# CWBudde/algo-dsp

Hardware: AMD Instinct MI355X
Metric: Msamples/sec, overlap-save conv 131072-tap IR @48kHz; achieved HBM GB/s (higher is better)
Workload: dtype f64

## Files before the change

### algo-dsp_amd/csrc/conv_long_kernels.hip

```cpp
#include "conv_long_kernels.hpp"

#include "conv_kernels.hpp"
#include "fft_device.hpp"

namespace adsp {

constexpr int N1 = kLongN1, N2 = kLongN2, W = kLongW;
constexpr int kColThreads = 256;
constexpr int kRowsPerInstr = kColThreads / W;
constexpr int FS = N1 + 1;
using ColPlan = FftPlan<N1, 16>;
constexpr int RV = 8;
using RowPlan = FftPlan<N2, RV>;
static_assert(ColPlan::T * (W / 2) == kColThreads, "a tile's transforms fill the workgroup");
static_assert(N1 % kRowsPerInstr == 0, "whole load rounds");
static_assert(ColPlan::T <= 64 && 64 % ColPlan::T == 0, "a column transform sits inside one wave");

__global__ __launch_bounds__(kColThreads) void k_long_cols_fwd(LongColArgs a) {
  __shared__ double2 lds[(W / 2) * FS];
  __shared__ double2 ltab[TwSplit<N1>::N];
  const int tid = threadIdx.x;
  const int item = xcd_remap(blockIdx.x, gridDim.x);
  constexpr int kTiles = N2 / W;
  const int tile = item % kTiles, cb = item / kTiles;
  const int c = cb / a.blocks, j = cb % a.blocks;
  const int col = tid % W, r0 = tid / W;
  const int64_t b0 = a.start + (int64_t)j * a.hop + tile * W + col;
  const double* x = a.x + (int64_t)c * a.x_stride;
  double in[N1 / kRowsPerInstr];
#pragma unroll
  for (int i = 0; i < N1 / kRowsPerInstr; ++i) {
    const int64_t idx = b0 + (int64_t)(r0 + kRowsPerInstr * i) * N2;
    in[i] = (idx >= 0 && idx < a.n) ? x[idx] : 0.0;
  }
  const TwLds<N1> tw = tw_lds_compute<N1>(ltab, tid, kColThreads);
  double* img = reinterpret_cast<double*>(lds + (col >> 1) * FS) + (col & 1);
#pragma unroll
  for (int i = 0; i < N1 / kRowsPerInstr; ++i) img[2 * lds_slot(r0 + kRowsPerInstr * i)] = in[i];
  __syncthreads();
  const int f = tid / ColPlan::T, t = tid % ColPlan::T;
  double2* my = lds + f * FS;
  double2 v[16];
#pragma unroll
  for (int s = 0; s < 16; ++s) v[s] = my[pass0_slot<N1, 16>(t, s)];
  __syncthreads();
  fft_run<N1, 16, true>(v, t, my, tw);
  __syncthreads();
#pragma unroll
  for (int s = 0; s < 16; ++s) my[last_pass_slot<N1, 16>(t, s)] = v[s];
  __syncthreads();
  const double2* zc = lds + (col >> 1) * FS;
  double2* T = a.T + (int64_t)cb * kLongRows * kLongPitch + tile * W + col;
#pragma unroll
  for (int i = 0; i <= N1 / 2 / kRowsPerInstr; ++i) {
    const int k1 = r0 + kRowsPerInstr * i;
    if (k1 <= N1 / 2) {
      const double2 zk = zc[lds_slot(k1)];
      const double2 zm = zc[lds_slot((N1 - k1) & (N1 - 1))];
      const double2 o = (col & 1) ? make_double2(0.5 * (zk.y + zm.y), 0.5 * (zm.x - zk.x))
                                  : make_double2(0.5 * (zk.x + zm.x), 0.5 * (zk.y - zm.y));
      st2<true>(T + (int64_t)k1 * kLongPitch, o);
    }
  }
}

__global__ __launch_bounds__(kColThreads) void k_long_cols_inv(LongColArgs a) {
  __shared__ double2 lds[(W / 2) * FS];
  __shared__ double2 ltab[TwSplit<N1>::N];
  const int tid = threadIdx.x;
  const int item = xcd_remap(blockIdx.x, gridDim.x);
  constexpr int kTiles = N2 / W;
  const int tile = item % kTiles, cb = item / kTiles;
  const int c = cb / a.blocks, j = cb % a.blocks;
  const int col = tid % W, r0 = tid / W;
  const double2* T = a.T + (int64_t)cb * kLongRows * kLongPitch + tile * W + col;
  constexpr int NI = N1 / 2 / kRowsPerInstr + 1;
  double2 in[NI];
#pragma unroll
  for (int i = 0; i < NI; ++i) {
    const int k1 = r0 + kRowsPerInstr * i;
    in[i] = k1 <= N1 / 2 ? ld2<true>(T + (int64_t)k1 * kLongPitch) : make_double2(0, 0);
  }
  const TwLds<N1> tw = tw_lds_compute<N1>(ltab, tid, kColThreads);
  double2* zc = lds + (col >> 1) * FS;
#pragma unroll
  for (int i = 0; i < NI; ++i) {
    const int k1 = r0 + kRowsPerInstr * i;
    const double px = __shfl_xor(in[i].x, 1);
    const double py = __shfl_xor(in[i].y, 1);
    if (k1 <= N1 / 2) {
      if (!(col & 1)) {
        const bool edge = k1 == 0 || k1 == N1 / 2;
        zc[lds_slot(k1)] = edge ? make_double2(in[i].x, px) : make_double2(in[i].x - py, in[i].y + px);
      } else if (k1 != 0 && k1 != N1 / 2) {
        zc[lds_slot(N1 - k1)] = make_double2(px + in[i].y, in[i].x - py);
      }
    }
  }
  __syncthreads();
  const int f = tid / ColPlan::T, t = tid % ColPlan::T;
  double2* my = lds + f * FS;
  double2 v[16];
#pragma unroll
  for (int s = 0; s < 16; ++s) v[s] = my[pass0_slot<N1, 16>(t, s)];
  wave_lds_sync();
  fft_run_wave<N1, 16, false>(v, t, my, tw);
  wave_lds_sync();
#pragma unroll
  for (int s = 0; s < 16; ++s) my[last_pass_slot<N1, 16>(t, s)] = v[s];
  __syncthreads();
  const double* img = reinterpret_cast<const double*>(zc) + (col & 1);
  double* y = a.y + (int64_t)c * a.y_stride;
  const int64_t o0 = (int64_t)j * a.hop - a.skip + tile * W + col;
  const int64_t lo = (int64_t)j * a.hop;
  const int64_t hi = a.out_len < lo + a.hop ? a.out_len : lo + a.hop;
#pragma unroll
  for (int i = 0; i < N1 / kRowsPerInstr; ++i) {
    const int r = r0 + kRowsPerInstr * i;
    const int64_t o = o0 + (int64_t)r * N2;
    if (o >= lo && o < hi) y[o] = img[2 * lds_slot(r)];
  }
}

constexpr int kRowThreads = RowPlan::T;
static_assert(RowPlan::NPASS == 4 && RowPlan::R0 == RV && RV == 8 && kRowThreads == 8 * 64,
              "k_long_rows: four radix-8 passes over eight waves of 64 lanes, wave = k0");

__device__ __forceinline__ double wave_bcast(double x, int l) {
  const int lo = __builtin_amdgcn_readlane(__double2loint(x), l);
  const int hi = __builtin_amdgcn_readlane(__double2hiint(x), l);
  return __hiloint2double(hi, lo);
}

constexpr int kRowWavesPerSimd = 2 * kRowThreads / 256;
template <bool BUILD>
__global__ __launch_bounds__(kRowThreads, kRowWavesPerSimd) void k_long_rows(LongRowArgs a) {
  __shared__ double2 lds[N2];
  __shared__ double2 ltab[TwSplit<N2>::N];
  __shared__ double2 wtab[kRowThreads];
  constexpr int T = kRowThreads;
  const int tid = threadIdx.x;
  const int lane = tid & 63;
  const int wv = __builtin_amdgcn_readfirstlane(tid >> 6);
  const int l0 = lane & 7, l1 = lane & 56;
  const int item = xcd_remap(blockIdx.x, gridDim.x);
  const int ncb = a.blocks * a.channels;
  const int cb = item % ncb, k1 = item / ncb;
  double2* row = a.T + ((int64_t)cb * kLongRows + k1) * kLongPitch;
  double2 v[RV];
#pragma unroll
  for (int s = 0; s < RV; ++s) v[s] = ld2<true>(row + tid + T * s);
  const TwLds<N2> tw = tw_lds_compute<N2>(ltab, tid, T);
  double2 rt[RV];
  {
    double2 r;
    sincospi(-2.0 * (double)(T * k1 * l0) / (double)kLongN, &r.y, &r.x);
#pragma unroll
    for (int s = 0; s < RV; ++s) rt[s] = make_double2(wave_bcast(r.x, s), wave_bcast(r.y, s));
  }
  {
    double2 w0;
    sincospi(-2.0 * (double)(k1 * tid) / (double)kLongN, &w0.y, &w0.x);
    wtab[tid] = w0;
#pragma unroll
    for (int s = 0; s < RV; ++s) v[s] = c_mul(v[s], c_mul(w0, rt[s]));
  }
  Dft<RV, true>::run(v);
#pragma unroll
  for (int r = 0; r < RV; ++r) lds[T * r + tid] = v[r];
  double2 h[BUILD ? 1 : RV];
  if constexpr (!BUILD) {
    const double2* hrow = a.H + ((int64_t)a.ir_index[cb / a.blocks] * kLongRows + k1) * kLongPitch;
#pragma unroll
    for (int s = 0; s < RV; ++s) h[s] = hrow[tid + T * s];
  }
  __syncthreads();
  double2* sl = lds + 64 * RV * wv;
  double2 w = twiddle_root<N2, RV, 8, true>(wv, tw);
#pragma unroll
  for (int r = 0; r < RV; ++r) v[r] = sl[64 * r + lane];
  twiddle_powers<RV>(v, w);
  Dft<RV, true>::run(v);
  wave_lds_sync();
#pragma unroll
  for (int r = 0; r < RV; ++r) sl[8 * l1 + 8 * r + l0] = v[r];
  w = twiddle_root<N2, RV, 64, true>(l1 + wv, tw);
  wave_lds_sync();
#pragma unroll
  for (int r = 0; r < RV; ++r) v[r] = sl[64 * r + lane];
  twiddle_powers<RV>(v, w);
  Dft<RV, true>::run(v);
  wave_lds_sync();
#pragma unroll
  for (int r = 0; r < RV; ++r) sl[64 * l0 + ((l1 + r) ^ l0)] = v[r];
  w = twiddle_root<N2, RV, 512, true>(64 * l0 + l1 + wv, tw);
  wave_lds_sync();
#pragma unroll
  for (int r = 0; r < RV; ++r) v[r] = sl[64 * r + (lane ^ r)];
  twiddle_powers<RV>(v, w);
  Dft<RV, true>::run(v);
  if constexpr (BUILD) {
    double2* out = a.Hout + ((int64_t)cb * kLongRows + k1) * kLongPitch;
#pragma unroll
    for (int s = 0; s < RV; ++s) out[tid + T * s] = c_scale(v[s], a.scale);
  } else {
#pragma unroll
    for (int s = 0; s < RV; ++s) v[s] = c_mul(v[s], h[s]);
    Dft<RV, false>::run(v);
    wave_lds_sync();
#pragma unroll
    for (int r = 0; r < RV; ++r) sl[64 * l0 + ((l1 + r) ^ l0)] = v[r];
    w = twiddle_root<N2, RV, 8, false>(l0, tw);
    wave_lds_sync();
#pragma unroll
    for (int r = 0; r < RV; ++r) v[r] = sl[64 * r + (lane ^ r)];
    twiddle_powers<RV>(v, w);
    Dft<RV, false>::run(v);
    wave_lds_sync();
#pragma unroll
    for (int r = 0; r < RV; ++r) sl[8 * l1 + 8 * r + l0] = v[r];
    w = twiddle_root<N2, RV, 64, false>(lane, tw);
    wave_lds_sync();
#pragma unroll
    for (int r = 0; r < RV; ++r) v[r] = sl[64 * r + lane];
    twiddle_powers<RV>(v, w);
    Dft<RV, false>::run(v);
    wave_lds_sync();
#pragma unroll
    for (int r = 0; r < RV; ++r) sl[64 * r + lane] = v[r];
    w = twiddle_root<N2, RV, 512, false>(tid, tw);
    const double2 w0 = wtab[tid];
    __syncthreads();
#pragma unroll
    for (int r = 0; r < RV; ++r) v[r] = lds[T * r + tid];
    twiddle_powers<RV>(v, w);
    Dft<RV, false>::run(v);
#pragma unroll
    for (int s = 0; s < RV; ++s) st2<true>(row + tid + T * s, c_mul(v[s], c_conj(c_mul(w0, rt[s]))));
  }
}

void launch_long_cols_fwd(const LongColArgs& a, hipStream_t s) {
  const unsigned items = (unsigned)a.channels * a.blocks * (N2 / W);
  timed_launch(k_long_cols_fwd, dim3(items), dim3(kColThreads), s, a);
}

void launch_long_rows(const LongRowArgs& a, bool build_h, hipStream_t s) {
  const unsigned items = (unsigned)a.channels * a.blocks * kLongRows;
  if (build_h)
    timed_launch(k_long_rows<true>, dim3(items), dim3(kRowThreads), s, a);
  else
    timed_launch(k_long_rows<false>, dim3(items), dim3(kRowThreads), s, a);
}

void launch_long_cols_inv(const LongColArgs& a, hipStream_t s) {
  const unsigned items = (unsigned)a.channels * a.blocks * (N2 / W);
  timed_launch(k_long_cols_inv, dim3(items), dim3(kColThreads), s, a);
}

}
```

### algo-dsp_amd/csrc/fft_device.hpp

```cpp
#pragma once

#include <hip/hip_runtime.h>

namespace adsp {

struct cplx {
  double x, y;
};

typedef double d2v_t __attribute__((ext_vector_type(2)));
template <bool NT>
__device__ __forceinline__ double2 ld2(const double2* p) {
  if constexpr (NT) {
    const d2v_t t = __builtin_nontemporal_load(reinterpret_cast<const d2v_t*>(p));
    return make_double2(t.x, t.y);
  } else {
    return *p;
  }
}
template <bool NT>
__device__ __forceinline__ void st2(double2* p, double2 v) {
  if constexpr (NT)
    __builtin_nontemporal_store(d2v_t{v.x, v.y}, reinterpret_cast<d2v_t*>(p));
  else
    *p = v;
}

__device__ __forceinline__ double2 c_add(double2 a, double2 b) { return make_double2(a.x + b.x, a.y + b.y); }
__device__ __forceinline__ double2 c_sub(double2 a, double2 b) { return make_double2(a.x - b.x, a.y - b.y); }
__device__ __forceinline__ double2 c_mul(double2 a, double2 b) {
  return make_double2(a.x * b.x - a.y * b.y, a.x * b.y + a.y * b.x);
}
__device__ __forceinline__ double2 c_conj(double2 a) { return make_double2(a.x, -a.y); }
__device__ __forceinline__ double2 c_scale(double2 a, double s) { return make_double2(a.x * s, a.y * s); }

__device__ constexpr double kCos16[16] = {
    1.0,
    0.92387953251128675613,
    0.70710678118654752440,
    0.38268343236508977173,
    0.0,
    -0.38268343236508977173,
    -0.70710678118654752440,
    -0.92387953251128675613,
    -1.0,
    -0.92387953251128675613,
    -0.70710678118654752440,
    -0.38268343236508977173,
    0.0,
    0.38268343236508977173,
    0.70710678118654752440,
    0.92387953251128675613,
};

template <int E, bool FWD>
__device__ __forceinline__ double2 tw16(double2 a) {
  constexpr int e = E & 15;
  constexpr double R2 = 0.70710678118654752440;
  if constexpr (e == 0) {
    return a;
  } else if constexpr (e == 4) {
    return FWD ? make_double2(a.y, -a.x) : make_double2(-a.y, a.x);
  } else if constexpr (e == 8) {
    return make_double2(-a.x, -a.y);
  } else if constexpr (e == 12) {
    return FWD ? make_double2(-a.y, a.x) : make_double2(a.y, -a.x);
  } else if constexpr (e == 2) {
    return FWD ? make_double2((a.x + a.y) * R2, (a.y - a.x) * R2) : make_double2((a.x - a.y) * R2, (a.y + a.x) * R2);
  } else if constexpr (e == 6) {
    return FWD ? make_double2((a.y - a.x) * R2, -(a.x + a.y) * R2) : make_double2(-(a.x + a.y) * R2, (a.x - a.y) * R2);
  } else if constexpr (e == 10) {
    return FWD ? make_double2(-(a.x + a.y) * R2, (a.x - a.y) * R2) : make_double2((a.y - a.x) * R2, -(a.x + a.y) * R2);
  } else if constexpr (e == 14) {
    return FWD ? make_double2((a.x - a.y) * R2, (a.y + a.x) * R2) : make_double2((a.x + a.y) * R2, (a.y - a.x) * R2);
  } else {
    constexpr double c = kCos16[e];
    constexpr double s0 = kCos16[(e + 12) & 15];
    constexpr double s = FWD ? -s0 : s0;
    return make_double2(a.x * c - a.y * s, a.x * s + a.y * c);
  }
}

template <int R, bool FWD>
struct Dft {
  template <int I = 0>
  __device__ static __forceinline__ void combine(double2* v, const double2* e, const double2* o) {
    if constexpr (I < R / 2) {
      const double2 t = tw16<I*(16 / R), FWD>(o[I]);
      v[I] = c_add(e[I], t);
      v[I + R / 2] = c_sub(e[I], t);
      combine<I + 1>(v, e, o);
    }
  }
  __device__ static __forceinline__ void run(double2* v) {
    double2 e[R / 2], o[R / 2];
#pragma unroll
    for (int i = 0; i < R / 2; ++i) {
      e[i] = v[2 * i];
      o[i] = v[2 * i + 1];
    }
    Dft<R / 2, FWD>::run(e);
    Dft<R / 2, FWD>::run(o);
    combine(v, e, o);
  }
};
template <bool FWD>
struct Dft<1, FWD> {
  __device__ static __forceinline__ void run(double2*) {}
};

__host__ __device__ constexpr int ilog2c(int v) { return v <= 1 ? 0 : 1 + ilog2c(v >> 1); }
template <int M, int V = 16>
struct FftPlan {
  static_assert(M >= 16 && M <= 8192 && (M & (M - 1)) == 0, "FFT size must be a power of two in [16, 8192]");
  static_assert(V == 4 || V == 8 || V == 16, "4, 8 or 16 values per thread");
  static constexpr int LOGV = ilog2c(V);
  static constexpr int LOG = ilog2c(M);
  static constexpr int NPASS = (LOG + LOGV - 1) / LOGV;
  static constexpr int R0 = 1 << (LOG - LOGV * (NPASS - 1));
  static constexpr int T = M / V;
  static constexpr int BLOCK = T > 256 ? T : 256;
  static constexpr int F = BLOCK / T;
  static constexpr int MP = M + (T < 16 ? T : 0);
  static constexpr int radix(int p) { return p == 0 ? R0 : V; }
  static constexpr int ns(int p) { return p == 0 ? 1 : R0 * (1 << (LOGV * (p - 1))); }
};

__device__ __forceinline__ int xcd_remap(int b, int G) {
  const int xcd = b & 7, r = b >> 3;
  const int q = G >> 3, rem = G & 7;
  return (xcd < rem) ? xcd * (q + 1) + r : rem * (q + 1) + (xcd - rem) * q + r;
}

#ifndef AD_LDS_SWZ
#define AD_LDS_SWZ 1
#endif
__device__ __forceinline__ int lds_slot(int i) {
#if AD_LDS_SWZ
  const int t = (i >> 3) & 15;
  return i ^ (int)((0xde0321fc12cfed30ull >> (4 * t)) & 15);
#else
  const int q = i >> 4;
  return i ^ ((q ^ ((q & 4) << 1)) & 15);
#endif
}
__device__ __forceinline__ int lds_slot_split(int swz_base, int off) { return swz_base ^ lds_slot(off); }
__device__ __forceinline__ int tw_slot(int i) { return i ^ ((i >> 3) & 7); }

struct TwGlobal {
  const double2* __restrict__ t;
  __device__ __forceinline__ double2 operator()(int e) const { return t[e]; }
};
template <int M>
struct TwSplit {
  static constexpr int S = (ilog2c(M) + 1) / 2;
  static constexpr int NLO = 1 << S;
  static constexpr int NHI = M >> S;
  static constexpr int N = NLO + NHI;
};
template <int M>
struct TwLds {
  const double2* lo;
  const double2* hi;
  __device__ __forceinline__ double2 operator()(int e) const {
    using Sp = TwSplit<M>;
    if constexpr (Sp::NHI == 1) return lo[tw_slot(e)];
    const double2 a = lo[tw_slot(e & (Sp::NLO - 1))];
    const double2 b = hi[e >> Sp::S];
    return c_mul(a, b);
  }
};
template <int M, int STRIDE = 1>
__device__ __forceinline__ TwLds<M> tw_lds_fill(double2* ltab, const double2* __restrict__ g, int tid, int nthreads) {
  using Sp = TwSplit<M>;
  for (int i = tid; i < Sp::N; i += nthreads) {
    if (i < Sp::NLO)
      ltab[tw_slot(i)] = g[i * STRIDE];
    else
      ltab[i] = g[((i - Sp::NLO) << Sp::S) * STRIDE];
  }
  return TwLds<M>{ltab, ltab + Sp::NLO};
}

template <int M>
__device__ __forceinline__ TwLds<M> tw_lds_compute(double2* ltab, int tid, int nthreads) {
  using Sp = TwSplit<M>;
  for (int i = tid; i < Sp::N; i += nthreads) {
    const int e = i < Sp::NLO ? i : ((i - Sp::NLO) << Sp::S);
    double sn, cs;
    sincospi(-2.0 * (double)e / (double)M, &sn, &cs);
    ltab[i < Sp::NLO ? tw_slot(i) : i] = make_double2(cs, sn);
  }
  return TwLds<M>{ltab, ltab + Sp::NLO};
}

template <int M, int R, int NS, bool FWD, class TW>
__device__ __forceinline__ void apply_twiddles(double2* v, int jb, const TW& tw) {
  if constexpr (NS > 1) {
    const int e = (jb & (NS - 1)) * (M / (NS * R));
    double2 w = tw(e);
    if (!FWD) w = c_conj(w);
    double2 wr = w;
#pragma unroll
    for (int r = 1; r < R; ++r) {
      v[r] = c_mul(v[r], wr);
      if (r + 1 < R) wr = c_mul(wr, w);
    }
  }
}

template <int M, int V, int P, bool FWD, class TW>
__device__ __forceinline__ void pass_compute_store(double2* v, int tid, double2* lds, const TW& twM) {
  using Plan = FftPlan<M, V>;
  constexpr int R = Plan::radix(P);
  constexpr int NS = Plan::ns(P);
  constexpr int NB = V / R;
#pragma unroll
  for (int b = 0; b < NB; ++b) {
    const int jb = tid + b * Plan::T;
    apply_twiddles<M, R, NS, FWD, TW>(v + b * R, jb, twM);
    Dft<R, FWD>::run(v + b * R);
  }
#pragma unroll
  for (int b = 0; b < NB; ++b) {
    const int jb = tid + b * Plan::T;
    const int base = (jb / NS) * NS * R + (jb & (NS - 1));
    const int sb = lds_slot(base);
#pragma unroll
    for (int r = 0; r < R; ++r) lds[lds_slot_split(sb, r * NS)] = v[b * R + r];
  }
}

template <int M, int V, int P>
__device__ __forceinline__ void pass_load(double2* v, int tid, const double2* lds) {
  using Plan = FftPlan<M, V>;
  constexpr int R = Plan::radix(P);
  constexpr int NB = V / R;
#pragma unroll
  for (int b = 0; b < NB; ++b) {
    const int jb = tid + b * Plan::T;
    const int sb = lds_slot(jb);
#pragma unroll
    for (int r = 0; r < R; ++r) v[b * R + r] = lds[lds_slot_split(sb, r * (M / R))];
  }
}

template <int M, int V = 16>
__device__ __forceinline__ int pass0_index(int tid, int s) {
  using Plan = FftPlan<M, V>;
  constexpr int R = Plan::R0;
  const int b = s / R, r = s % R;
  return tid + b * Plan::T + r * (M / R);
}

template <int M, int V = 16>
__device__ __forceinline__ int pass0_slot(int tid, int s) {
  using Plan = FftPlan<M, V>;
  constexpr int R = Plan::R0;
  const int b = s / R, r = s % R;
  return lds_slot_split(lds_slot(tid + b * Plan::T), r * (M / R));
}

template <int M, int V, bool FWD, int P = 1, class TW>
__device__ __forceinline__ void run_middle_passes(double2* v, int tid, double2* lds, const TW& twM) {
  using Plan = FftPlan<M, V>;
  if constexpr (P < Plan::NPASS) {
    __syncthreads();
    pass_load<M, V, P>(v, tid, lds);
    if constexpr (P + 1 < Plan::NPASS) {
      __syncthreads();
      pass_compute_store<M, V, P, FWD, TW>(v, tid, lds, twM);
      run_middle_passes<M, V, FWD, P + 1, TW>(v, tid, lds, twM);
    }
  }
}

template <int M, int V, bool FWD, class TW>
__device__ __forceinline__ void last_pass_compute(double2* v, int tid, const TW& twM) {
  using Plan = FftPlan<M, V>;
  constexpr int P = Plan::NPASS - 1;
  constexpr int R = Plan::radix(P);
  constexpr int NS = Plan::ns(P);
  constexpr int NB = V / R;
#pragma unroll
  for (int b = 0; b < NB; ++b) {
    const int jb = tid + b * Plan::T;
    apply_twiddles<M, R, NS, FWD, TW>(v + b * R, jb, twM);
    Dft<R, FWD>::run(v + b * R);
  }
}

template <int M, int V = 16>
__device__ __forceinline__ int last_pass_index(int tid, int s) {
  using Plan = FftPlan<M, V>;
  constexpr int P = Plan::NPASS - 1;
  constexpr int R = Plan::radix(P);
  constexpr int NS = Plan::ns(P);
  const int b = s / R, r = s % R;
  const int jb = tid + b * Plan::T;
  return (jb / NS) * NS * R + (jb & (NS - 1)) + r * NS;
}

template <int M, int V = 16>
__device__ __forceinline__ int last_pass_slot(int tid, int s) {
  using Plan = FftPlan<M, V>;
  constexpr int P = Plan::NPASS - 1;
  constexpr int R = Plan::radix(P);
  constexpr int NS = Plan::ns(P);
  const int b = s / R, r = s % R;
  const int jb = tid + b * Plan::T;
  return lds_slot_split(lds_slot((jb / NS) * NS * R + (jb & (NS - 1))), r * NS);
}

template <int M, int V, bool FWD, class TW>
__device__ __forceinline__ void fft_run(double2* v, int tid, double2* lds, const TW& twM) {
  using Plan = FftPlan<M, V>;
  if constexpr (Plan::NPASS > 1) {
    pass_compute_store<M, V, 0, FWD, TW>(v, tid, lds, twM);
    run_middle_passes<M, V, FWD, 1, TW>(v, tid, lds, twM);
  }
  last_pass_compute<M, V, FWD, TW>(v, tid, twM);
}

__device__ __forceinline__ void wave_lds_sync() {
  __builtin_amdgcn_fence(__ATOMIC_RELEASE, "wavefront");
  __builtin_amdgcn_wave_barrier();
  __builtin_amdgcn_fence(__ATOMIC_ACQUIRE, "wavefront");
}

template <int M, int R, int NS, bool FWD, class TW>
__device__ __forceinline__ double2 twiddle_root(int jb, const TW& tw) {
  static_assert(NS > 1, "pass 0 has no twiddles");
  const double2 w = tw((jb & (NS - 1)) * (M / (NS * R)));
  return FWD ? w : c_conj(w);
}
template <int R>
__device__ __forceinline__ void twiddle_powers(double2* v, double2 w) {
  double2 wr = w;
#pragma unroll
  for (int r = 1; r < R; ++r) {
    v[r] = c_mul(v[r], wr);
    if (r + 1 < R) wr = c_mul(wr, w);
  }
}

template <int M, int V, bool FWD, int P = 1, class TW>
__device__ __forceinline__ void run_middle_passes_wave(double2* v, int tid, double2* lds, const TW& twM) {
  using Plan = FftPlan<M, V>;
  if constexpr (P < Plan::NPASS) {
    wave_lds_sync();
    pass_load<M, V, P>(v, tid, lds);
    if constexpr (P + 1 < Plan::NPASS) {
      wave_lds_sync();
      pass_compute_store<M, V, P, FWD, TW>(v, tid, lds, twM);
      run_middle_passes_wave<M, V, FWD, P + 1, TW>(v, tid, lds, twM);
    }
  }
}
template <int M, int V, bool FWD, class TW>
__device__ __forceinline__ void fft_run_wave(double2* v, int tid, double2* lds, const TW& twM) {
  using Plan = FftPlan<M, V>;
  static_assert(Plan::T <= 64 && 64 % Plan::T == 0, "the transform's threads must sit inside one wave");
  if constexpr (Plan::NPASS > 1) {
    pass_compute_store<M, V, 0, FWD, TW>(v, tid, lds, twM);
    run_middle_passes_wave<M, V, FWD, 1, TW>(v, tid, lds, twM);
  }
  last_pass_compute<M, V, FWD, TW>(v, tid, twM);
}

template <int M, int V, bool FWD, int P = 1, class TW>
__device__ __forceinline__ void run_middle_passes_active(double2* v, int tid, double2* lds, const TW& twM, bool active) {
  using Plan = FftPlan<M, V>;
  if constexpr (P < Plan::NPASS) {
    __syncthreads();
    if (active) pass_load<M, V, P>(v, tid, lds);
    if constexpr (P + 1 < Plan::NPASS) {
      __syncthreads();
      if (active) pass_compute_store<M, V, P, FWD, TW>(v, tid, lds, twM);
      run_middle_passes_active<M, V, FWD, P + 1, TW>(v, tid, lds, twM, active);
    }
  }
}
template <int M, int V, bool FWD, class TW>
__device__ __forceinline__ void fft_run_active(double2* v, int tid, double2* lds, const TW& twM, bool active) {
  using Plan = FftPlan<M, V>;
  if constexpr (Plan::NPASS > 1) {
    if (active) pass_compute_store<M, V, 0, FWD, TW>(v, tid, lds, twM);
    run_middle_passes_active<M, V, FWD, 1, TW>(v, tid, lds, twM, active);
  }
  if (active) last_pass_compute<M, V, FWD, TW>(v, tid, twM);
}

}
```

Measured before the change: 90140.

## Halve column-FFT LDS footprint by exchanging real and imaginary parts in separate passes

The column forward and inverse kernels now keep a real-valued (double) LDS image instead of a complex one. Each FFT exchange pass stores and loads the real and imaginary halves in two rounds through a new swizzled 8-byte slot map. Lane-pair data movement uses DPP swaps instead of __shfl_xor, and the launch bounds ask for four workgroups per CU. The aim is to cut LDS per workgroup so more workgroups fit on a CU and overlap memory latency. In exchange it doubles the LDS round-trips and barriers per pass and adds register pressure.

```diff
diff --git a/algo-dsp_amd/csrc/conv_long_kernels.hip b/algo-dsp_amd/csrc/conv_long_kernels.hip
--- a/algo-dsp_amd/csrc/conv_long_kernels.hip
+++ b/algo-dsp_amd/csrc/conv_long_kernels.hip
@@ -8,16 +8,32 @@
 constexpr int N1 = kLongN1, N2 = kLongN2, W = kLongW;
 constexpr int kColThreads = 256;
 constexpr int kRowsPerInstr = kColThreads / W;
-constexpr int FS = N1 + 1;
 using ColPlan = FftPlan<N1, 16>;
 constexpr int RV = 8;
 using RowPlan = FftPlan<N2, RV>;
 static_assert(ColPlan::T * (W / 2) == kColThreads, "a tile's transforms fill the workgroup");
 static_assert(N1 % kRowsPerInstr == 0, "whole load rounds");
 static_assert(ColPlan::T <= 64 && 64 % ColPlan::T == 0, "a column transform sits inside one wave");
-
-__global__ __launch_bounds__(kColThreads) void k_long_cols_fwd(LongColArgs a) {
-  __shared__ double2 lds[(W / 2) * FS];
+constexpr int kColFS = N1 + 2;
+constexpr int kColWgPerCu = 4;
+static_assert(kColWgPerCu * ((W / 2) * kColFS * 8 + TwSplit<N1>::N * 16) <= 160 * 1024, "the CU's LDS holds the workgroups");
+static_assert(N1 <= 512, "lds_slot8 maps nine-bit rows");
+
+__device__ __forceinline__ double lane_pair_swap(double x) {
+  const int lo = __builtin_amdgcn_update_dpp(0, __double2loint(x), 0xB1, 0xF, 0xF, false);
+  const int hi = __builtin_amdgcn_update_dpp(0, __double2hiint(x), 0xB1, 0xF, 0xF, false);
+  return __hiloint2double(hi, lo);
+}
+
+constexpr int kDealt = N1 / kRowsPerInstr / 2;
+__device__ __forceinline__ double* dealt_at(double* img, int sb8, int k) { return slot8_at(img, sb8, 2 * kRowsPerInstr * k); }
+
+__device__ __forceinline__ double* mirror_at(double* img, int sm8, int r0, int i) {
+  return r0 ? slot8_at(img, sm8, N1 - kRowsPerInstr * (i + 1)) : slot8_at(img, sm8, (N1 - kRowsPerInstr * i) & (N1 - 1));
+}
+
+__global__ __launch_bounds__(kColThreads, kColWgPerCu) void k_long_cols_fwd(LongColArgs a) {
+  __shared__ double lds[(W / 2) * kColFS];
   __shared__ double2 ltab[TwSplit<N1>::N];
   const int tid = threadIdx.x;
   const int item = xcd_remap(blockIdx.x, gridDim.x);
@@ -25,6 +41,7 @@
   const int tile = item % kTiles, cb = item / kTiles;
   const int c = cb / a.blocks, j = cb % a.blocks;
   const int col = tid % W, r0 = tid / W;
+  const bool odd = col & 1;
   const int64_t b0 = a.start + (int64_t)j * a.hop + tile * W + col;
   const double* x = a.x + (int64_t)c * a.x_stride;
   double in[N1 / kRowsPerInstr];
@@ -34,38 +51,67 @@
     in[i] = (idx >= 0 && idx < a.n) ? x[idx] : 0.0;
   }
   const TwLds<N1> tw = tw_lds_compute<N1>(ltab, tid, kColThreads);
-  double* img = reinterpret_cast<double*>(lds + (col >> 1) * FS) + (col & 1);
-#pragma unroll
-  for (int i = 0; i < N1 / kRowsPerInstr; ++i) img[2 * lds_slot(r0 + kRowsPerInstr * i)] = in[i];
-  __syncthreads();
+#pragma unroll
+  for (int k = 0; k < kDealt; ++k) {
+    const double got = lane_pair_swap(odd ? in[2 * k] : in[2 * k + 1]);
+    if (odd)
+      in[2 * k] = got;
+    else
+      in[2 * k + 1] = got;
+  }
+  double* zc = lds + (col >> 1) * kColFS;
+  const int sd = 8 * lds_slot8(r0 + kRowsPerInstr * (int)odd);
   const int f = tid / ColPlan::T, t = tid % ColPlan::T;
-  double2* my = lds + f * FS;
+  double* my = lds + f * kColFS;
   double2 v[16];
 #pragma unroll
-  for (int s = 0; s < 16; ++s) v[s] = my[pass0_slot<N1, 16>(t, s)];
-  __syncthreads();
-  fft_run<N1, 16, true>(v, t, my, tw);
-  __syncthreads();
-#pragma unroll
-  for (int s = 0; s < 16; ++s) my[last_pass_slot<N1, 16>(t, s)] = v[s];
-  __syncthreads();
-  const double2* zc = lds + (col >> 1) * FS;
+  for (int k = 0; k < kDealt; ++k) *dealt_at(zc, sd, k) = in[2 * k];
+  __syncthreads();
+#pragma unroll
+  for (int s = 0; s < 16; ++s) v[s].x = *pass0_at<N1, 16>(my, t, s);
+  __syncthreads();
+#pragma unroll
+  for (int k = 0; k < kDealt; ++k) *dealt_at(zc, lds_fresh(sd), k) = in[2 * k + 1];
+  __syncthreads();
+#pragma unroll
+  for (int s = 0; s < 16; ++s) v[s].y = *pass0_at<N1, 16>(my, lds_fresh(t), s);
+  wave_lds_sync();
+  fft_run_wave_split<N1, 16, true>(v, t, my, tw);
+  wave_lds_sync();
+  constexpr int NI = N1 / 2 / kRowsPerInstr + 1;
+  const int sk = 8 * lds_slot8(r0), sm = 8 * lds_slot8(r0 ? kRowsPerInstr - r0 : 0);
+  double part[NI];
+#pragma unroll
+  for (int s = 0; s < 16; ++s) *last_pass_at<N1, 16>(my, t, s) = v[s].x;
+  __syncthreads();
+#pragma unroll
+  for (int i = 0; i < NI; ++i) {
+    if (r0 + kRowsPerInstr * i <= N1 / 2) {
+      const double zkx = *slot8_at(zc, sk, kRowsPerInstr * i);
+      const double zmx = *mirror_at(zc, sm, r0, i);
+      part[i] = odd ? zmx - zkx : zkx + zmx;
+      asm volatile("" : "+v"(part[i]));
+    }
+  }
+  __syncthreads();
+#pragma unroll
+  for (int s = 0; s < 16; ++s) *last_pass_at<N1, 16>(my, lds_fresh(t), s) = v[s].y;
+  __syncthreads();
   double2* T = a.T + (int64_t)cb * kLongRows * kLongPitch + tile * W + col;
 #pragma unroll
-  for (int i = 0; i <= N1 / 2 / kRowsPerInstr; ++i) {
+  for (int i = 0; i < NI; ++i) {
     const int k1 = r0 + kRowsPerInstr * i;
     if (k1 <= N1 / 2) {
-      const double2 zk = zc[lds_slot(k1)];
-      const double2 zm = zc[lds_slot((N1 - k1) & (N1 - 1))];
-      const double2 o = (col & 1) ? make_double2(0.5 * (zk.y + zm.y), 0.5 * (zm.x - zk.x))
-                                  : make_double2(0.5 * (zk.x + zm.x), 0.5 * (zk.y - zm.y));
+      const double zky = *slot8_at(zc, lds_fresh(sk), kRowsPerInstr * i);
+      const double zmy = *mirror_at(zc, lds_fresh(sm), lds_fresh(r0), i);
+      const double2 o = odd ? make_double2(0.5 * (zky + zmy), 0.5 * part[i]) : make_double2(0.5 * part[i], 0.5 * (zky - zmy));
       st2<true>(T + (int64_t)k1 * kLongPitch, o);
     }
   }
 }
 
-__global__ __launch_bounds__(kColThreads) void k_long_cols_inv(LongColArgs a) {
-  __shared__ double2 lds[(W / 2) * FS];
+__global__ __launch_bounds__(kColThreads, kColWgPerCu) void k_long_cols_inv(LongColArgs a) {
+  __shared__ double lds[(W / 2) * kColFS];
   __shared__ double2 ltab[TwSplit<N1>::N];
   const int tid = threadIdx.x;
   const int item = xcd_remap(blockIdx.x, gridDim.x);
@@ -73,6 +119,7 @@
   const int tile = item % kTiles, cb = item / kTiles;
   const int c = cb / a.blocks, j = cb % a.blocks;
   const int col = tid % W, r0 = tid / W;
+  const bool odd = col & 1;
   const double2* T = a.T + (int64_t)cb * kLongRows * kLongPitch + tile * W + col;
   constexpr int NI = N1 / 2 / kRowsPerInstr + 1;
   double2 in[NI];
@@ -82,34 +129,69 @@
     in[i] = k1 <= N1 / 2 ? ld2<true>(T + (int64_t)k1 * kLongPitch) : make_double2(0, 0);
   }
   const TwLds<N1> tw = tw_lds_compute<N1>(ltab, tid, kColThreads);
-  double2* zc = lds + (col >> 1) * FS;
+  double* zc = lds + (col >> 1) * kColFS;
+  const int sz = 8 * lds_slot8(odd ? (kRowsPerInstr - r0) & (kRowsPerInstr - 1) : r0);
+  const int f = tid / ColPlan::T, t = tid % ColPlan::T;
+  double* my = lds + f * kColFS;
+  double2 v[16];
 #pragma unroll
   for (int i = 0; i < NI; ++i) {
     const int k1 = r0 + kRowsPerInstr * i;
-    const double px = __shfl_xor(in[i].x, 1);
-    const double py = __shfl_xor(in[i].y, 1);
+    const bool edge = k1 == 0 || k1 == N1 / 2;
+    const double got = lane_pair_swap(odd ? in[i].y : in[i].x);
+    double* zo = odd ? mirror_at(zc, sz, r0, i) : slot8_at(zc, sz, kRowsPerInstr * i);
     if (k1 <= N1 / 2) {
-      if (!(col & 1)) {
-        const bool edge = k1 == 0 || k1 == N1 / 2;
-        zc[lds_slot(k1)] = edge ? make_double2(in[i].x, px) : make_double2(in[i].x - py, in[i].y + px);
-      } else if (k1 != 0 && k1 != N1 / 2) {
-        zc[lds_slot(N1 - k1)] = make_double2(px + in[i].y, in[i].x - py);
-      }
+      if (!odd)
+        *zo = edge ? in[i].x : in[i].x - got;
+      else if (!edge)
+        *zo = got + in[i].y;
     }
   }
   __syncthreads();
-  const int f = tid / ColPlan::T, t = tid % ColPlan::T;
-  double2* my = lds + f * FS;
-  double2 v[16];
-#pragma unroll
-  for (int s = 0; s < 16; ++s) v[s] = my[pass0_slot<N1, 16>(t, s)];
-  wave_lds_sync();
-  fft_run_wave<N1, 16, false>(v, t, my, tw);
-  wave_lds_sync();
-#pragma unroll
-  for (int s = 0; s < 16; ++s) my[last_pass_slot<N1, 16>(t, s)] = v[s];
-  __syncthreads();
-  const double* img = reinterpret_cast<const double*>(zc) + (col & 1);
+#pragma unroll
+  for (int s = 0; s < 16; ++s) v[s].x = *pass0_at<N1, 16>(my, t, s);
+  __syncthreads();
+#pragma unroll
+  for (int i = 0; i < NI; ++i) {
+    const int k1 = r0 + kRowsPerInstr * i;
+    const bool edge = k1 == 0 || k1 == N1 / 2;
+    const double got = lane_pair_swap(odd ? in[i].x : in[i].y);
+    const int szy = lds_fresh(sz);
+    double* zo = odd ? mirror_at(zc, szy, lds_fresh(r0), i) : slot8_at(zc, szy, kRowsPerInstr * i);
+    if (k1 <= N1 / 2) {
+      if (!odd)
+        *zo = edge ? got : in[i].y + got;
+      else if (!edge)
+        *zo = in[i].x - got;
+    }
+  }
+  __syncthreads();
+#pragma unroll
+  for (int s = 0; s < 16; ++s) v[s].y = *pass0_at<N1, 16>(my, lds_fresh(t), s);
+  wave_lds_sync();
+  fft_run_wave_split<N1, 16, false>(v, t, my, tw);
+  wave_lds_sync();
+  const int sd = 8 * lds_slot8(r0 + kRowsPerInstr * (int)odd);
+  double out[N1 / kRowsPerInstr];
+#pragma unroll
+  for (int s = 0; s < 16; ++s) *last_pass_at<N1, 16>(my, t, s) = v[s].x;
+  __syncthreads();
+#pragma unroll
+  for (int k = 0; k < kDealt; ++k) out[2 * k] = *dealt_at(zc, sd, k);
+  __syncthreads();
+#pragma unroll
+  for (int s = 0; s < 16; ++s) *last_pass_at<N1, 16>(my, lds_fresh(t), s) = v[s].y;
+  __syncthreads();
+#pragma unroll
+  for (int k = 0; k < kDealt; ++k) out[2 * k + 1] = *dealt_at(zc, lds_fresh(sd), k);
+#pragma unroll
+  for (int k = 0; k < kDealt; ++k) {
+    const double got = lane_pair_swap(odd ? out[2 * k] : out[2 * k + 1]);
+    if (odd)
+      out[2 * k] = got;
+    else
+      out[2 * k + 1] = got;
+  }
   double* y = a.y + (int64_t)c * a.y_stride;
   const int64_t o0 = (int64_t)j * a.hop - a.skip + tile * W + col;
   const int64_t lo = (int64_t)j * a.hop;
@@ -118,7 +200,7 @@
   for (int i = 0; i < N1 / kRowsPerInstr; ++i) {
     const int r = r0 + kRowsPerInstr * i;
     const int64_t o = o0 + (int64_t)r * N2;
-    if (o >= lo && o < hi) y[o] = img[2 * lds_slot(r)];
+    if (o >= lo && o < hi) y[o] = out[i];
   }
 }
 
diff --git a/algo-dsp_amd/csrc/fft_device.hpp b/algo-dsp_amd/csrc/fft_device.hpp
--- a/algo-dsp_amd/csrc/fft_device.hpp
+++ b/algo-dsp_amd/csrc/fft_device.hpp
@@ -368,6 +368,152 @@
   last_pass_compute<M, V, FWD, TW>(v, tid, twM);
 }
 
+constexpr int kSlot8Swz[9] = {2, 0, 8, 0, 3, 6, 1, 9, 0};
+constexpr int lds_slot8_ref(int n) {
+  int m = n;
+  for (int j = 0; j < 9; ++j)
+    if ((n >> j) & 1) m ^= kSlot8Swz[j];
+  return m;
+}
+constexpr unsigned long long lds_slot8_table() {
+  unsigned long long t = 0;
+  for (int i = 0; i < 16; ++i) t |= (unsigned long long)(lds_slot8_ref(16 * i) ^ (16 * i)) << (4 * i);
+  return t;
+}
+__host__ __device__ constexpr int lds_slot8(int n) {
+  return n ^ ((n & 5) << 1) ^ (int)((lds_slot8_table() >> (4 * ((n >> 4) & 15))) & 15);
+}
+constexpr bool lds_slot8_matches() {
+  for (int n = 0; n < 512; ++n)
+    if (lds_slot8(n) != lds_slot8_ref(n)) return false;
+  return true;
+}
+static_assert(lds_slot8_matches(), "lds_slot8 is the bit map of kSlot8Swz for nine-bit elements");
+
+__device__ __forceinline__ double* slot8_at(double* img, int sb8, int off) {
+  const int s = lds_slot8(off);
+  return reinterpret_cast<double*>(reinterpret_cast<char*>(img) + (sb8 ^ ((s & 15) << 3)) + ((s & ~15) << 3));
+}
+__device__ __forceinline__ const double* slot8_at(const double* img, int sb8, int off) {
+  return slot8_at(const_cast<double*>(img), sb8, off);
+}
+
+template <bool Y>
+__device__ __forceinline__ double& c_part(double2& v) {
+  if constexpr (Y)
+    return v.y;
+  else
+    return v.x;
+}
+
+__device__ __forceinline__ int lds_fresh(int x) {
+  asm volatile("" : "+v"(x));
+  return x;
+}
+
+template <bool WAVE>
+__device__ __forceinline__ void split_sync() {
+  if constexpr (WAVE)
+    wave_lds_sync();
+  else
+    __syncthreads();
+}
+
+template <int M, int V, int P, bool FWD, class TW>
+__device__ __forceinline__ void pass_compute(double2* v, int tid, const TW& twM) {
+  using Plan = FftPlan<M, V>;
+  constexpr int R = Plan::radix(P);
+  constexpr int NS = Plan::ns(P);
+  constexpr int NB = V / R;
+#pragma unroll
+  for (int b = 0; b < NB; ++b) {
+    const int jb = tid + b * Plan::T;
+    apply_twiddles<M, R, NS, FWD, TW>(v + b * R, jb, twM);
+    Dft<R, FWD>::run(v + b * R);
+  }
+}
+
+template <int M, int V, int P, bool Y>
+__device__ __forceinline__ void pass_store_split(double2* v, int tid, double* img) {
+  static_assert(M <= 512, "lds_slot8 maps nine-bit elements");
+  tid = lds_fresh(tid);
+  using Plan = FftPlan<M, V>;
+  constexpr int R = Plan::radix(P);
+  constexpr int NS = Plan::ns(P);
+  constexpr int NB = V / R;
+#pragma unroll
+  for (int b = 0; b < NB; ++b) {
+    const int jb = tid + b * Plan::T;
+    const int sb8 = 8 * lds_slot8((jb / NS) * NS * R + (jb & (NS - 1)));
+#pragma unroll
+    for (int r = 0; r < R; ++r) *slot8_at(img, sb8, r * NS) = c_part<Y>(v[b * R + r]);
+  }
+}
+
+template <int M, int V, int P, bool Y>
+__device__ __forceinline__ void pass_load_split(double2* v, int tid, const double* img) {
+  static_assert(M <= 512, "lds_slot8 maps nine-bit elements");
+  tid = lds_fresh(tid);
+  using Plan = FftPlan<M, V>;
+  constexpr int R = Plan::radix(P);
+  constexpr int NB = V / R;
+#pragma unroll
+  for (int b = 0; b < NB; ++b) {
+    const int jb = tid + b * Plan::T;
+    const int sb8 = 8 * lds_slot8(jb);
+#pragma unroll
+    for (int r = 0; r < R; ++r) c_part<Y>(v[b * R + r]) = *slot8_at(img, sb8, r * (M / R));
+  }
+}
+
+template <int M, int V = 16>
+__device__ __forceinline__ double* pass0_at(double* img, int tid, int s) {
+  using Plan = FftPlan<M, V>;
+  constexpr int R = Plan::R0;
+  const int b = s / R, r = s % R;
+  return slot8_at(img, 8 * lds_slot8(tid + b * Plan::T), r * (M / R));
+}
+template <int M, int V = 16>
+__device__ __forceinline__ double* last_pass_at(double* img, int tid, int s) {
+  using Plan = FftPlan<M, V>;
+  constexpr int P = Plan::NPASS - 1;
+  constexpr int R = Plan::radix(P);
+  constexpr int NS = Plan::ns(P);
+  const int b = s / R, r = s % R;
+  const int jb = tid + b * Plan::T;
+  return slot8_at(img, 8 * lds_slot8((jb / NS) * NS * R + (jb & (NS - 1))), r * NS);
+}
+
+template <int M, int V, bool FWD, bool WAVE, int P = 0, class TW>
+__device__ __forceinline__ void run_passes_split(double2* v, int tid, double* img, const TW& twM) {
+  using Plan = FftPlan<M, V>;
+  if constexpr (P + 1 < Plan::NPASS) {
+    pass_compute<M, V, P, FWD, TW>(v, tid, twM);
+    pass_store_split<M, V, P, false>(v, tid, img);
+    split_sync<WAVE>();
+    pass_load_split<M, V, P + 1, false>(v, tid, img);
+    split_sync<WAVE>();
+    pass_store_split<M, V, P, true>(v, tid, img);
+    split_sync<WAVE>();
+    pass_load_split<M, V, P + 1, true>(v, tid, img);
+    if constexpr (P + 2 < Plan::NPASS) split_sync<WAVE>();
+    run_passes_split<M, V, FWD, WAVE, P + 1, TW>(v, tid, img, twM);
+  }
+}
+
+template <int M, int V, bool FWD, class TW>
+__device__ __forceinline__ void fft_run_split(double2* v, int tid, double* img, const TW& twM) {
+  run_passes_split<M, V, FWD, false, 0, TW>(v, tid, img, twM);
+  last_pass_compute<M, V, FWD, TW>(v, tid, twM);
+}
+template <int M, int V, bool FWD, class TW>
+__device__ __forceinline__ void fft_run_wave_split(double2* v, int tid, double* img, const TW& twM) {
+  using Plan = FftPlan<M, V>;
+  static_assert(Plan::T <= 64 && 64 % Plan::T == 0, "the transform's threads must sit inside one wave");
+  run_passes_split<M, V, FWD, true, 0, TW>(v, tid, img, twM);
+  last_pass_compute<M, V, FWD, TW>(v, tid, twM);
+}
+
 template <int M, int V, bool FWD, int P = 1, class TW>
 __device__ __forceinline__ void run_middle_passes_active(double2* v, int tid, double2* lds, const TW& twM, bool active) {
   using Plan = FftPlan<M, V>;
```

Measured after the change: 86220. 0.957x the previous value.
